# Jittor/JDet

Hardware: AMD Instinct MI355X
Metric: img/s S2ANet-R50-FPN train step, 1024x1024 synthetic tiles (higher is better)
Workload: dtype f32; 1 GPU; s2anet_train; model=S2ANet-R50-FPN (configs/s2anet/s2anet_r50_fpn_1x_dota.py), global_batch=2, tile=1024x1024, gts_per_image=64, optimizer=SGD mom 0.9 wd 1e-4 clip 35 + StepLR warm-up (the config's lr), parallelism=dp1 (DDP, RCCL all-reduce)

## Files before the change

jdet_amd/_lib.py:

```python
import ctypes
import os
import subprocess

import torch

_HERE = os.path.dirname(os.path.abspath(__file__))
CSRC = os.path.join(_HERE, "csrc")
LIB_PATH = os.path.join(CSRC, "libjdet_hip.so")

_i, _f, _p, _sz, _l = ctypes.c_int, ctypes.c_float, ctypes.c_void_p, ctypes.c_size_t, ctypes.c_long



class BnParams(ctypes.Structure):
    _fields_ = [("weight", _p), ("bias", _p), ("mean", _p), ("var", _p), ("eps", _f)]


class ConvEpilogue(ctypes.Structure):
    _fields_ = [("mode", _i), ("affine", _i), ("relu", _i), ("bn", BnParams), ("residual", _p), ("grad_out", _p),
                ("act", _p), ("sums", _p)]


class BnSumsJob(ctypes.Structure):
    _fields_ = [("partial", _p), ("rows", _l), ("C", _i), ("gamma", _p), ("grad_gamma", _p), ("grad_beta", _p)]


class GaussianLossParams(ctypes.Structure):
    _fields_ = [("kind", _i), ("fun", _i), ("tau", _f), ("alpha", _f), ("normalize", _i), ("sqrt_dist", _i),
                ("beta", _f), ("eps", _f), ("decode_pred", _i), ("decode_target", _i), ("means", _f * 5),
                ("stds", _f * 5), ("wh_ratio_clip", _f)]


GD_KINDS = {"gwd": 0, "kld": 1, "jd": 2, "kld_symmax": 3, "kld_symmin": 4, "gwd_v1": 5, "kld_v1": 6, "bcd_v1": 7,
            "kfiou": 8}
GD_FUNS = {"none": 0, "": 0, None: 0, "log1p": 1, "sqrt": 2, "ln": 3, "exp": 4}

EPI_FORWARD, EPI_ADD, EPI_MASK = 0, 1, 2

SIGNATURES = {
    "jdet_version": (_i, []),
    "jdet_nchw_to_nhwc": (_i, [_p, _i, _i, _i, _i, _p, _p]),
    "jdet_nhwc_to_nchw": (_i, [_p, _i, _i, _i, _i, _p, _p]),
    "jdet_roi_align_forward": (_i, [_i, _p, _i, _i, _i, _i, _p, _i, _i, _i, _f, _i, _i, _p, _p, _p]),
    "jdet_roi_align_forward_cl_roi": (_i, [_i, _p, _i, _i, _i, _i, _p, _i, _i, _i, _f, _i, _i, _p, _p, _p]),
    "jdet_roi_align_forward_cl_workspace": (_sz, [_i, _i, _i]),
    "jdet_roi_align_forward_cl": (_i, [_i, _p, _i, _i, _i, _i, _p, _i, _i, _i, _f, _i, _i, _p, _p, _sz, _p]),
    "jdet_roi_align_forward_reference": (_i, [_i, _p, _i, _i, _i, _i, _p, _i, _i, _i, _f, _i, _i, _p, _p, _p]),
    "jdet_roi_align_forward_cl_reference": (_i, [_i, _p, _i, _i, _i, _i, _p, _i, _i, _i, _f, _i, _i, _p, _p, _sz, _p]),
    "jdet_roi_align_backward_cl": (_i, [_i, _p, _p, _i, _i, _i, _i, _i, _i, _i, _f, _i, _i, _p, _p, _sz, _i, _p]),
    "jdet_roi_align_backward_clean_bytes": (_sz, [_i] * 9),
    "jdet_roi_align_backward_plan_bytes": (_sz, [_i] * 8),
    "jdet_roi_align_backward_plan": (_i, [_i, _p, _i, _i, _i, _i, _i, _i, _f, _i, _p, _sz, _p]),
    "jdet_roi_align_backward_cl_planned": (_i, [_i, _p, _i, _i, _i, _i, _i, _i, _i, _i, _p, _p, _sz, _p]),
    "jdet_roi_align_backward_workspace": (_sz, [_i] * 9),
    "jdet_roi_align_backward": (_i, [_i, _p, _p, _i, _i, _i, _i, _i, _i, _i, _f, _i, _i, _p, _p, _p, _sz, _p]),
    "jdet_roi_spatial_order": (_i, [_p, _i, _i, _f, _i, _i, _i, _p, _p, _p]),
    "jdet_box_iou_rotated": (_i, [_p, _i, _p, _i, _i, _i, _i, _p, _p]),
    "jdet_nms_rotated_workspace": (_sz, [_i]),
    "jdet_nms_rotated": (_i, [_p, _i, _i, _p, _f, _i, _i, _p, _p, _sz, _p]),
    "jdet_upsample_add_nhwc_forward": (_i, [_p, _p, _i, _i, _i, _i, _i, _i, _f, _p, _p]),
    "jdet_upsample_add_nhwc_backward": (_i, [_p, _i, _i, _i, _i, _i, _i, _f, _p, _p]),
    "jdet_zero_fill": (_i, [_p, _sz, _p]),
    "jdet_graph_replace_memset_nodes": (_i, [_p, ctypes.POINTER(ctypes.c_int)]),
    "jdet_sum_squares_workspace": (_sz, []),
    "jdet_sum_squares": (_i, [_p, _sz, _i, _p, _p, _sz, _p]),
    "jdet_normalize_u8_nhwc": (_i, [_p, _p, _i, _i, _i, _p, _p, _i, _p, _p]),
    "jdet_feature_refine_forward": (_i, [_p, _p, _i, _i, _i, _i, _f, _i, _p, _p]),
    "jdet_feature_refine_backward_workspace": (_sz, [_i] * 5),
    "jdet_feature_refine_backward": (_i, [_p, _p, _i, _i, _i, _i, _f, _i, _p, _p, _sz, _p]),
    "jdet_poly_iou": (_i, [_p, _i, _i, _p, _i, _i, _i, _p, _p]),
    "jdet_nms_poly": (_i, [_p, _i, _i, _p, _f, _i, _p, _p, _sz, _p]),
    "jdet_bbox_overlaps_hbb": (_i, [_p, _i, _p, _i, _i, _i, _i, _f, _p, _p, _p]),
    "jdet_nms_labeled": (_i, [_p, _i, _i, _p, _f, _i, _i, _i, _i, _p, _p, _sz, _p]),
    "jdet_deform_im2col": (_i, [_p, _p] + [_i] * 13 + [_p, _p]),
    "jdet_deform_col2im": (_i, [_p, _p] + [_i] * 13 + [_p, _p]),
    "jdet_deform_col2im_coord": (_i, [_p, _p, _p] + [_i] * 13 + [_p, _p]),
    "jdet_modulated_deform_im2col": (_i, [_p, _p, _p] + [_i] * 13 + [_p, _p]),
    "jdet_modulated_deform_col2im": (_i, [_p, _p, _p] + [_i] * 13 + [_p, _p]),
    "jdet_modulated_deform_col2im_coord": (_i, [_p, _p, _p, _p] + [_i] * 13 + [_p, _p, _p]),
    "jdet_deform_psroi_pool_forward": (_i, [_p, _p, _p] + [_i] * 6 + [_f] + [_i] * 5 + [_f, _i, _p, _p, _p]),
    "jdet_deform_psroi_pool_backward": (_i, [_p, _p, _p, _p, _p] + [_i] * 6 + [_f] + [_i] * 5 + [_f, _i, _p, _p, _p]),
    "jdet_deform_im2col_nhwc": (_i, [_p, _p] + [_i] * 12 + [_p, _p]),
    "jdet_deform_col2im_nhwc_workspace": (_sz, [_i] * 12),
    "jdet_deform_col2im_nhwc": (_i, [_p, _p] + [_i] * 12 + [_p, _p, _sz, _p]),
    "jdet_convex_iou": (_i, [_p, _i, _p, _i, _p, _p]),
    "jdet_convex_giou": (_i, [_p, _p, _i, _p, _p]),
    "jdet_min_area_bbox": (_i, [_p, _i, _p, _p]),
    "jdet_convex_sort": (_i, [_p, _p, _i, _i, _i, _p, _p]),
    "jdet_conv3x3_igemm_supported": (_i, [_i, _i]),
    "jdet_conv3x3_igemm_forward": (_i, [_p, _i, _i, _i, _i, _p, _i, _p, _i, _p, _p, _i, _p, _p, _sz, _p]),
    "jdet_conv3x3_igemm_workspace": (_sz, [_i] * 5),
    "jdet_conv3x3_wgrad_supported": (_i, [_i, _i]),
    "jdet_conv3x3_wgrad": (_i, [_p, _p, _p, _i, _i, _i, _i, _i, _p, _i, _p]),
    "jdet_conv_bn_supported": (_i, [_i] * 4),
    "jdet_conv_bn_workspace": (_sz, [_i] * 7),
    "jdet_conv_bn_sums_rows": (_sz, [_i] * 9),
    "jdet_conv_bn_forward": (_i, [_p, _i, _i, _i, _i, _p, _i, _i, _i, ctypes.POINTER(ConvEpilogue), _i, _p, _p, _sz, _p]),
    "jdet_conv_dgrad_weights": (_i, [_p, _i, _i, _p]),
    "jdet_conv_wgrad": (_i, [_p, _p, _i, _i, _i, _i, _i, _i, _i, _p, _i, _p]),
    "jdet_bn_act_backward_from_output_rows": (_sz, [_l, _i]),
    "jdet_bn_act_backward_from_output": (_i, [_p, _p, _p, _p, _l, _i, _p, _p, _p, _p, _f, _p, _p, _sz, _p]),
    "jdet_bn_sums_finish": (_i, [ctypes.POINTER(BnSumsJob), _i, _p]),
    "jdet_sigmoid_focal_loss_workspace": (_sz, []),
    "jdet_sigmoid_focal_loss": (_i, [_p, _p, _p, _l, _i, _f, _f, _p, _p, _p, _sz, _p]),
    "jdet_smooth_l1_loss": (_i, [_p, _p, _p, _l, _f, _p, _p, _p, _sz, _p]),
    "jdet_sigmoid_focal_loss_level": (_i, [_p, _p, _l, _l, _p, _l, _l, _l, _i, _f, _f, _p, _f, _p, _p, _p, _sz, _p]),
    "jdet_smooth_l1_loss_level": (_i, [_p, _p, _l, _l, _p, _l, _l, _l, _i, _f, _p, _f, _p, _p, _p, _sz, _p]),
    "jdet_loss_grad_scale": (_i, [_p, _l, _p, _p, _f, _p, _p]),
    "jdet_gaussian_loss_level": (_i, [_p, _p, _l, _l, _p, _l, _l, _p, _l, _l, ctypes.POINTER(GaussianLossParams), _p, _f,
                                      _p, _p, _p, _sz, _p]),
    "jdet_level_pack_nhwc": (_i, [_p, _p, _p, _i, _i, _i, _i, _i, _p, _p]),
    "jdet_align_conv_offset": (_i, [_p, _i, _i, _i, _f, _i, _p, _p]),
    "jdet_frozen_bn_act_forward": (_i, [_p, _p, _l, _i, _p, _p, _p, _p, _f, _i, _p, _p]),
    "jdet_frozen_bn_act_backward_workspace": (_sz, [_l, _i]),
    "jdet_frozen_bn_act_backward": (_i, [_p, _p, _p, _l, _i, _p, _p, _p, _p, _f, _i, _p, _p, _p, _p, _p, _sz, _p]),
    "jdet_bias_act_backward": (_i, [_p, _p, _l, _i, _i, _p, _p, _p, _sz, _p]),
    "jdet_channel_sum_workspace": (_sz, [_l, _i]),
    "jdet_channel_sum": (_i, [_p, _l, _i, _p, _p, _sz, _p]),
    "jdet_arf_forward": (_i, [_p, _p] + [_i] * 6 + [_p, _p]),
    "jdet_arf_backward": (_i, [_p, _p] + [_i] * 6 + [_p, _p]),
    "jdet_arf_forward_cl": (_i, [_p, _p] + [_i] * 6 + [_p, _p]),
    "jdet_arf_backward_cl": (_i, [_p, _p] + [_i] * 6 + [_p, _p]),
    "jdet_rip_forward": (_i, [_p, _l, _i, _i, _p, _p]),
    "jdet_rip_backward": (_i, [_p, _p, _p, _l, _i, _i, _p, _p]),
    "jdet_delta2bbox_rotated": (_i, [_p, _p, _i, _i, _p, _p, _f, _p, _p]),
    "jdet_bbox2delta_rotated": (_i, [_p, _p, _i, _p, _p, _p, _p]),
    "jdet_midpoint_offset_decode": (_i, [_p, _p, _l, _p, _p, _f, _p, _p]),
    "jdet_midpoint_offset_encode": (_i, [_p, _p, _l, _p, _p, _p, _p]),
    "jdet_oriented_delta_decode": (_i, [_p, _p, _l, _i, _p, _p, _f, _p, _p]),
    "jdet_oriented_delta_encode": (_i, [_p, _p, _l, _p, _p, _p, _p]),
    "jdet_gliding_targets": (_i, [_p, _p, _l, _p, _p, _p, _p, _p, _p]),
    "jdet_gliding_decode": (_i, [_p, _p, _p, _p, _l, _i, _p, _p, _f, _f, _f, _f, _p, _p, _p]),
    "jdet_gv_delta_encode": (_i, [_p, _p, _l, _p, _p, _p, _p]),
    "jdet_gv_delta_decode": (_i, [_p, _p, _l, _i, _p, _p, _f, _f, _f, _p, _p]),
    "jdet_anchor_targets_rotated": (_i, [_p, _p, _p, _p, _i, _i, _p, _p, _f, _p, _p, _p, _p, _p, _p]),
    "jdet_anchor_targets_rotated_boxes": (_i, [_p, _p, _p, _i, _i, _f, _p, _p, _p, _p, _p, _p]),
    "jdet_obb2hbb2obb": (_i, [_p, _i, _i, _p, _p]),
    "jdet_assign_max_iou_workspace": (_sz, [_i]),
    "jdet_assign_max_iou": (_i, [_p, _i, _i, _f, _f, _f, _f, _i, _i, _p, _i, _p, _p, _p, _p, _sz, _p]),
}

ATSS_SIGNATURES = {
    "jdet_atss_assign_workspace": (_sz, [_i, _i, _i, _i]),
    "jdet_atss_assign": (_i, [_p, _i, _i, _p, _i, _p, _i, _p, _p, _i, _i, _p, _p, _p, _p, _sz, _p]),
}

ROWS_SIGNATURES = {
    "jdet_rows_nonzero_workspace": (_sz, [_i, _i, _i]),
    "jdet_rows_nonzero": (_i, [_p, _i, _i, _i, _i, _p, _p, _p, _p, _p, _sz, _p]),
    "jdet_conv3x3_rows_supported": (_i, [_i, _i]),
    "jdet_conv3x3_wgrad_rows_workers": (_i, [_i, _i]),
    "jdet_conv3x3_wgrad_rows": (_i, [_p, _p, _p, _p, _i, _i, _i, _i, _i, _p, _p]),
    "jdet_conv3x3_dgrad_rows": (_i, [_p, _p, _p, _p, _i, _i, _i, _i, _i, _i, _p, _p]),
}

ROWS_FWD_SIGNATURES = {
    "jdet_rows_from_flags_workspace": (_sz, [_i, _i, _i]),
    "jdet_rows_from_flags": (_i, [_p, _i, _i, _i, _p, _p, _p, _p, _p, _sz, _p]),
    "jdet_conv3x3_rows_forward_supported": (_i, [_i, _i]),
    "jdet_conv3x3_rows_forward": (_i, [_p, _p, _p, _i, _p, _p, _p, _i, _i, _i, _i, _i, _i, _p, _p]),
}

FCOS_SIGNATURES = {
    "jdet_fcos_targets": (_i, [_p, _p, _i, _p, _p, _p, _i, _i, _i, _i, _i, _f, _p, _p, _p, _p, _p]),
    "jdet_poly_iou_loss": (_i, [_p, _p, _p, _l, _i, _f, _p, _p, _p]),
}

REPPOINTS_SIGNATURES = {
    "jdet_convex_point_assign_workspace": (_sz, [_i, _i]),
    "jdet_convex_point_assign": (_i, [_p, _i, _i, _p, _p, _i, _p, _p, _p, _i, _i, _f, _i, _i, _p, _p, _p, _sz, _p]),
    "jdet_convex_giou_loss": (_i, [_p, _p, _p, _p, _l, _p, _p, _p]),
}

H2RBOX_SIGNATURES = {
    "jdet_rotate_crop": (_i, [_p, _i, _i, _i, _i, _i, _i, _f, _f, _i, _p, _p]),
    "jdet_h2rbox_aug_loss_forward": (_i, [_p, _i, _p, _p, _p, _p, _p, _i, _i, _f, _f, _f, _i, _i, _f, _f, _f, _p, _p, _p]),
    "jdet_h2rbox_aug_loss_backward": (_i, [_p, _i, _p, _p, _p, _p, _p, _i, _i, _f, _f, _f, _i, _i, _f, _f, _f, _p, _p, _p,
                                           _p, _p, _p, _p, _p]),
}

LD_SIGNATURES = {
    "jdet_dist_integral": (_i, [_p, _l, _i, _f, _f, _f, _f, _p, _p]),
    "jdet_dist_bbox_loss_level": (_i, [_p, _p, _l, _l, _p, _l, _l, _l, _i, _f, _f, _f, _f, _f, _p, _f, _p, _p, _p, _sz, _p]),
    "jdet_kd_kl_div_level_forward": (_i, [_p, _p, _p, _l, _l, _l, _i, _f, _f, _p, _p, _p, _sz, _p]),
    "jdet_kd_kl_div_level_backward": (_i, [_p, _p, _p, _l, _l, _l, _i, _f, _f, _p, _p, _p, _p]),
}

_lib = None

REFERENCE_SORT = 0


def build(force=False, verbose=False):
    cmd = ["make", "-C", CSRC, "-j8"] + (["-B"] if force else [])
    r = subprocess.run(cmd, capture_output=True, text=True)
    if r.returncode != 0:
        raise RuntimeError("building libjdet_hip.so failed:\n" + r.stdout[-4000:] + r.stderr[-4000:])
    if verbose:
        print(r.stdout[-2000:])
    return LIB_PATH


def lib():
    global _lib
    if _lib is None:
        if not os.path.exists(LIB_PATH):
            raise RuntimeError(
                "jdet_amd: %s not found.  Build it with `python -c 'import __graft_entry__ as g; g.build()'` "
                "or `make -C jdet_amd/csrc` (needs hipcc).  There is no CPU fallback." % LIB_PATH)
        l = ctypes.CDLL(LIB_PATH)
        for name, (res, args) in list(SIGNATURES.items()) + list(ATSS_SIGNATURES.items()) + list(ROWS_SIGNATURES.items()) + \
                list(ROWS_FWD_SIGNATURES.items()) + list(FCOS_SIGNATURES.items()) + list(REPPOINTS_SIGNATURES.items()) + \
                list(H2RBOX_SIGNATURES.items()) + list(LD_SIGNATURES.items()):
            fn = getattr(l, name)
            fn.restype = res
            fn.argtypes = args
        _lib = l
    return _lib


class JDetHipError(RuntimeError):
    pass


_ERR = {-1: "bad argument", -2: "unsupported shape", -3: "workspace too small"}


def check(status, what):
    if status != 0:
        msg = _ERR.get(status, "hipError_t %d" % status)
        raise JDetHipError("%s failed: %s" % (what, msg))


def stream_ptr(t=None):
    if t is not None and t.is_cuda and t.device.index != torch.cuda.current_device():
        torch.cuda.set_device(t.device)
    return torch.cuda.current_stream(t.device if t is not None else None).cuda_stream


def need_device(*tensors):
    for t in tensors:
        if t is None:
            continue
        if not t.is_cuda:
            raise JDetHipError(
                "jdet_amd ops run only on a HIP device (got a %s tensor); there is no CPU fallback "
                "in the product path" % t.device)


def f32c(t):
    if t.dtype != torch.float32:
        t = t.float()
    return t.contiguous()


def vec5(v):
    return (ctypes.c_float * 5)(*[float(x) for x in v])


def vecn(v, n):
    v = [float(x) for x in v]
    assert len(v) == n
    return (ctypes.c_float * n)(*v)


def ptr(t):
    return t.data_ptr() if t is not None and t.numel() > 0 else None


def zero_(t):
    need_device(t)
    nbytes = t.numel() * t.element_size()
    if nbytes % 4 or not (t.is_contiguous() or t.is_contiguous(memory_format=torch.channels_last)):
        return t.zero_()
    check(lib().jdet_zero_fill(ptr(t), nbytes, stream_ptr(t)), "jdet_zero_fill")
    return t


def norm2(flat, ws=None):
    need_device(flat)
    n = flat.numel()
    wsb = lib().jdet_sum_squares_workspace()
    if ws is None:
        ws = torch.empty((wsb,), dtype=torch.uint8, device=flat.device)
    out = torch.empty((1,), dtype=torch.float32, device=flat.device)
    check(lib().jdet_sum_squares(ptr(flat), n, 1, ptr(out), ptr(ws), ws.numel(), stream_ptr(flat)), "jdet_sum_squares")
    return out[0]


def new_graph():
    return torch.cuda.CUDAGraph(keep_graph=True)


def harden_graph(g):
    n = ctypes.c_int(0)
    check(lib().jdet_graph_replace_memset_nodes(ctypes.c_void_p(g.raw_cuda_graph()), ctypes.byref(n)),
          "jdet_graph_replace_memset_nodes")
    return n.value
```

jdet_amd/ops/conv_igemm.py:

```python
import os
import weakref

import torch

from jdet_amd import _lib as L


def supported(cin, cout):
    return bool(L.lib().jdet_conv3x3_igemm_supported(int(cin), int(cout)))


def weight_krsc(weight):
    return L.f32c(weight.permute(0, 2, 3, 1))


def conv3x3_nhwc(x_nhwc, w_krsc, bias=None, relu=False, rowmask=None, offset=None, tile=0):
    L.need_device(x_nhwc, w_krsc, bias, rowmask, offset)
    N, H, W, Cin = x_nhwc.shape
    Cout = w_krsc.shape[0]
    if w_krsc.shape[1:] != (3, 3, Cin):
        raise ValueError("weight %r does not match input channels %d" % (tuple(w_krsc.shape), Cin))
    if offset is not None and tuple(offset.shape) != (N, 18, H, W):
        raise ValueError("offset must be (N, 18, H, W), got %r" % (tuple(offset.shape),))
    x_nhwc, w_krsc = L.f32c(x_nhwc), L.f32c(w_krsc)
    y = torch.empty((N, H, W, Cout), dtype=torch.float32, device=x_nhwc.device)
    ws, nbytes = None, 0
    if tile == 0 and offset is None:
        nbytes = L.lib().jdet_conv3x3_igemm_workspace(N, H, W, Cin, Cout)
        if nbytes:
            ws = torch.empty((nbytes,), dtype=torch.uint8, device=x_nhwc.device)
    L.check(L.lib().jdet_conv3x3_igemm_forward(
        L.ptr(x_nhwc), N, H, W, Cin, L.ptr(w_krsc), Cout,
        L.ptr(L.f32c(bias)) if bias is not None else None, int(bool(relu)),
        L.ptr(L.f32c(rowmask)) if rowmask is not None else None,
        L.ptr(L.f32c(offset)) if offset is not None else None,
        int(tile), L.ptr(y), L.ptr(ws), nbytes, L.stream_ptr(x_nhwc)), "jdet_conv3x3_igemm_forward")
    return y


def conv3x3(x, weight, bias=None, relu=False, offset=None, tile=0):
    y = conv3x3_nhwc(L.f32c(x.permute(0, 2, 3, 1)), weight_krsc(weight), bias, relu, None, offset, tile)
    return y.permute(0, 3, 1, 2)


MIN_POSITIONS = int(os.environ.get("JDET_CONV_MIN_POS", "1"))
DEFORM_MIN_POSITIONS = 32768
ENABLED = os.environ.get("JDET_CONV_IGEMM", "1") == "1"
TRAIN = os.environ.get("JDET_CONV_IGEMM_TRAIN", "1") == "1"

def needs_grad(*tensors):
    return torch.is_grad_enabled() and any(t is not None and t.requires_grad for t in tensors)


def preferred(x, weight, min_positions=None):
    if not (ENABLED and x.is_cuda and x.dtype == torch.float32 and weight.dtype == torch.float32 and x.dim() == 4):
        return False
    N, Cin, H, W = x.shape
    if tuple(weight.shape[1:]) != (Cin, 3, 3) or not supported(Cin, weight.shape[0]):
        return False
    if N * H * W * max(Cin, weight.shape[0]) >= 2 ** 30:
        return False
    return N * H * W >= (MIN_POSITIONS if min_positions is None else min_positions)


def wgrad_supported(cin, cout):
    return bool(L.lib().jdet_conv3x3_wgrad_supported(int(cin), int(cout)))


def conv3x3_wgrad_nhwc(x_nhwc, gy_nhwc, offset=None, out=None, ksplit=0, rows=None):
    L.need_device(x_nhwc, gy_nhwc, offset, out)
    N, H, W, Cin = x_nhwc.shape
    Cout = gy_nhwc.shape[3]
    if tuple(gy_nhwc.shape[:3]) != (N, H, W):
        raise ValueError("gy %r does not match x %r" % (tuple(gy_nhwc.shape), tuple(x_nhwc.shape)))
    if offset is not None and tuple(offset.shape) != (N, 18, H, W):
        raise ValueError("offset must be (N, 18, H, W), got %r" % (tuple(offset.shape),))
    x_nhwc, gy_nhwc = L.f32c(x_nhwc), L.f32c(gy_nhwc)
    if out is None:
        out = torch.zeros((Cout, 3, 3, Cin), dtype=torch.float32, device=x_nhwc.device)
    elif tuple(out.shape) != (Cout, 3, 3, Cin) or not out.is_contiguous() or out.dtype != torch.float32:
        raise ValueError("out must be a contiguous fp32 (Cout, 3, 3, Cin) tensor")
    L.check(_wgrad_call(x_nhwc, gy_nhwc, offset, N, H, W, Cin, Cout, L.ptr(out), ksplit, rows), "jdet_conv3x3_wgrad")
    return out


def conv3x3_wgrad(x, gy, offset=None, ksplit=0):
    gw = conv3x3_wgrad_nhwc(L.f32c(x.permute(0, 2, 3, 1)), L.f32c(gy.permute(0, 2, 3, 1)), offset, None, ksplit)
    return gw.permute(0, 3, 1, 2)


WGRAD = os.environ.get("JDET_CONV_WGRAD", "1") == "1"
def _wgrad_call(x_nhwc, gy_nhwc, offset, N, H, W, Cin, Cout, out_ptr, ksplit, rows=None):
    if rows is not None:
        if offset is not None:
            raise ValueError("the row list belongs to the plain form")
        return L.lib().jdet_conv3x3_wgrad_rows(L.ptr(x_nhwc), L.ptr(gy_nhwc), L.ptr(rows[0]), rows[1], N, H, W, Cin, Cout,
                                               out_ptr, L.stream_ptr(x_nhwc))
    return L.lib().jdet_conv3x3_wgrad(L.ptr(x_nhwc), L.ptr(gy_nhwc), L.ptr(L.f32c(offset)) if offset is not None else None,
                                      N, H, W, Cin, Cout, out_ptr, int(ksplit), L.stream_ptr(x_nhwc))


_GW_ACC = {}


def shared_wgrad(weight, x_nhwc, gy_nhwc, offset=None, rows=None):
    tid = torch._C._current_graph_task_id()
    key = weight.data_ptr()
    Cout, Cin = weight.shape[0], weight.shape[1]
    hit = _GW_ACC.get(key)
    stream = torch.cuda.current_stream(x_nhwc.device).cuda_stream if x_nhwc.is_cuda else 0
    if hit is not None and len(hit) > 3 and hit[3] != stream:
        hit = None
    if tid >= 0 and hit is not None and hit[0] == tid and hit[2] == (Cout, Cin, x_nhwc.device):
        N, H, W, _ = x_nhwc.shape
        x_nhwc, gy_nhwc = L.f32c(x_nhwc), L.f32c(gy_nhwc)
        L.check(_wgrad_call(x_nhwc, gy_nhwc, offset, N, H, W, Cin, Cout, hit[1], 0, rows), "jdet_conv3x3_wgrad")
        return None
    buf = conv3x3_wgrad_nhwc(x_nhwc, gy_nhwc, offset, rows=rows)
    if tid >= 0 and (_GW_ACC.get(key) is None or _GW_ACC[key][0] != tid):
        _GW_ACC[key] = (tid, buf.data_ptr(), (Cout, Cin, x_nhwc.device), stream)
    return buf.permute(0, 3, 1, 2)


_FLIPPED = {}
DGRAD = os.environ.get("JDET_CONV_IGEMM_DGRAD", "0") == "1"


class _WeightRef:

    def __init__(self, w):
        self.ref = weakref.ref(w)

    @property
    def weight(self):
        return self.ref()


_DGRAD_BANKS = {}


def dgrad_weight(weight):
    st = None
    if weight.is_cuda and weight.dtype == torch.float32 and weight.permute(0, 2, 3, 1).is_contiguous() \
            and not torch.cuda.is_current_stream_capturing():
        from jdet_amd.ops.conv_bn import DgradBank
        st = _DGRAD_BANKS.setdefault(weight.device, {"items": {}, "bank": None})
        it = st["items"].get(id(weight))
        if it is None or it.weight is not weight or any(v.weight is None for v in st["items"].values()):
            live = {k: v for k, v in st["items"].items() if v.weight is not None}
            it = live[id(weight)] = _WeightRef(weight)
            st["items"] = live
            st["bank"] = DgradBank(list(live.values()))
        return st["bank"].get(it)
    if weight.is_cuda and torch.cuda.is_current_stream_capturing():
        st = _DGRAD_BANKS.get(weight.device)
        it = st["items"].get(id(weight)) if st else None
        if it is not None and it.weight is weight and st["bank"].buf is not None:
            return st["bank"].get(it)
    key, stamp = id(weight), (weight.data_ptr(), weight._version)
    hit = _FLIPPED.get(key)
    if hit is None or hit[0] != stamp:
        hit = (stamp, weight.detach().flip(2, 3).permute(1, 2, 3, 0).contiguous())
        _FLIPPED[key] = hit
    return hit[1]


BIAS_ACT_BWD = os.environ.get("JDET_BIAS_ACT_BWD", "1") == "1"
_BWD_WS = {}


def _bias_bwd_supported(c):
    q = c // 4
    return c % 4 == 0 and ((q <= 256 and 256 % q == 0) or 256 < q <= 1024)


def bias_act_backward(g, y, relu):
    N, C, H, W = g.shape
    if (BIAS_ACT_BWD and not relu and g.is_cuda and g.dtype == torch.float32 and not _bias_bwd_supported(C)
            and C <= 256 and N * H * W > 0):
        gn = L.f32c(g.permute(0, 2, 3, 1))
        P = N * H * W
        nbytes = L.lib().jdet_channel_sum_workspace(P, C)
        ws = torch.empty((nbytes,), dtype=torch.uint8, device=g.device)
        gb = torch.empty((C,), dtype=torch.float32, device=g.device)
        L.check(L.lib().jdet_channel_sum(L.ptr(gn), P, C, L.ptr(gb), L.ptr(ws), nbytes, L.stream_ptr(gn)),
                "jdet_channel_sum")
        return g, gb
    if not (BIAS_ACT_BWD and g.is_cuda and g.dtype == torch.float32 and _bias_bwd_supported(C) and N * H * W > 0):
        gp = torch.ops.aten.threshold_backward(g, y, 0) if relu else g
        return gp, gp.sum((0, 2, 3))
    gn = L.f32c(g.permute(0, 2, 3, 1))
    P = N * H * W
    nbytes = L.lib().jdet_frozen_bn_act_backward_workspace(P, C)
    if torch.cuda.is_current_stream_capturing():
        ws = torch.empty((max(nbytes, 1),), dtype=torch.uint8, device=g.device)
    else:
        key = (g.device.index, torch.cuda.current_stream(g.device).cuda_stream)
        ws = _BWD_WS.get(key)
        if ws is None or ws.numel() < nbytes:
            while len(_BWD_WS) >= 8:
                _BWD_WS.pop(next(iter(_BWD_WS)))
            ws = _BWD_WS[key] = torch.empty((max(nbytes, 1 << 20),), dtype=torch.uint8, device=g.device)
    gb = torch.empty((C,), dtype=torch.float32, device=g.device)
    gp = torch.empty_like(gn) if relu else gn
    yn = L.f32c(y.permute(0, 2, 3, 1)) if relu else None
    L.check(L.lib().jdet_bias_act_backward(L.ptr(gn), L.ptr(yn), P, C, int(bool(relu)), L.ptr(gp) if relu else None,
                                           L.ptr(gb), L.ptr(ws), ws.numel(), L.stream_ptr(gn)),
            "jdet_bias_act_backward")
    return gp.permute(0, 3, 1, 2), gb


ROWS = os.environ.get("JDET_CONV_ROWS", "1") == "1"
_ROWS_WS = {}


def wgrad_rows_workers(cin, cout):
    return int(L.lib().jdet_conv3x3_wgrad_rows_workers(int(cin), int(cout)))


def rows_supported(cin, cout):
    return bool(L.lib().jdet_conv3x3_rows_supported(int(cin), int(cout)))


def _rows_scratch(nbytes, device):
    if torch.cuda.is_current_stream_capturing():
        return torch.empty((nbytes,), dtype=torch.uint8, device=device)
    key = (device.index, torch.cuda.current_stream(device).cuda_stream)
    ws = _ROWS_WS.get(key)
    if ws is None or ws.numel() < nbytes:
        while len(_ROWS_WS) >= 8:
            _ROWS_WS.pop(next(iter(_ROWS_WS)))
        ws = _ROWS_WS[key] = torch.empty((max(nbytes, 1 << 20),), dtype=torch.uint8, device=device)
    return ws


def rows_nonzero(g_nhwc, scratch=None):
    L.need_device(g_nhwc)
    N, H, W, C = g_nhwc.shape
    P = N * H * W
    g_nhwc = L.f32c(g_nhwc)
    wsb = L.lib().jdet_rows_nonzero_workspace(N, H, W)
    total = 8 * P + 16 + wsb + P
    buf = _rows_scratch(total, g_nhwc.device) if scratch is None else scratch
    rows = buf[:4 * P].view(torch.int32)
    drows = buf[4 * P:8 * P].view(torch.int32)
    counts = buf[8 * P:8 * P + 8].view(torch.int32)
    ws = buf[8 * P + 16:8 * P + 16 + wsb]
    flags = buf[8 * P + 16 + wsb:total]
    L.check(L.lib().jdet_rows_nonzero(L.ptr(g_nhwc), N, H, W, C, L.ptr(flags), L.ptr(rows), L.ptr(drows), L.ptr(counts),
                                      L.ptr(ws), wsb, L.stream_ptr(g_nhwc)), "jdet_rows_nonzero")
    return flags, rows, drows, counts


def conv3x3_dgrad_rows_nhwc(gy_nhwc, wd_crsk, rows, count_ptr, out=None):
    L.need_device(gy_nhwc, wd_crsk, rows, out)
    N, H, W, Cout = gy_nhwc.shape
    Cin = wd_crsk.shape[0]
    if tuple(wd_crsk.shape) != (Cin, 3, 3, Cout) or not wd_crsk.is_contiguous():
        raise ValueError("wd must be a contiguous (Cin, 3, 3, Cout) tensor, got %r" % (tuple(wd_crsk.shape),))
    gy_nhwc = L.f32c(gy_nhwc)
    zero = out is None
    if zero:
        out = torch.empty((N, H, W, Cin), dtype=torch.float32, device=gy_nhwc.device)
    L.check(L.lib().jdet_conv3x3_dgrad_rows(L.ptr(gy_nhwc), L.ptr(wd_crsk), L.ptr(rows), count_ptr, N, H, W, Cin, Cout,
                                            int(zero), L.ptr(out), L.stream_ptr(gy_nhwc)), "jdet_conv3x3_dgrad_rows")
    return out


def _rows_dgrad_weight(weight):
    if torch.cuda.is_current_stream_capturing() or not weight.is_cuda:
        return weight.detach().flip(2, 3).permute(1, 2, 3, 0).contiguous()
    wd = dgrad_weight(weight)
    st = _DGRAD_BANKS.get(weight.device)
    if st is None or st["bank"] is None or id(weight) not in st["items"]:
        return dgrad_weight_fresh(weight)
    tid = torch._C._current_graph_task_id()
    if tid < 0 or st.get("pass") != tid:
        st["bank"].refresh()
        st["pass"] = tid
    return wd


def dgrad_weight_fresh(weight):
    return weight.detach().flip(2, 3).permute(1, 2, 3, 0).contiguous()


def _rows_backward(g, x, weight, need_x, need_w):
    gn, xn = L.f32c(g.permute(0, 2, 3, 1)), L.f32c(x.permute(0, 2, 3, 1))
    _, rows, drows, counts = rows_nonzero(gn)
    gx = gw = None
    if need_w:
        gw = shared_wgrad(weight, xn, gn, rows=(rows, counts.data_ptr()))
    if need_x:
        gx = conv3x3_dgrad_rows_nhwc(gn, _rows_dgrad_weight(weight), drows, counts.data_ptr() + 4).permute(0, 3, 1, 2)
    return gx, gw


ROWS_FWD = os.environ.get("JDET_CONV_ROWS_FWD", "1") == "1"


def rows_forward_supported(cin, cout):
    return bool(L.lib().jdet_conv3x3_rows_forward_supported(int(cin), int(cout)))


def rows_from_flags(flags, N, H, W):
    L.need_device(flags)
    P = N * H * W
    if flags.numel() != P or flags.element_size() != 1 or not flags.is_contiguous():
        raise ValueError("flags must be %d contiguous bytes, got %r %s" % (P, tuple(flags.shape), flags.dtype))
    wsb = L.lib().jdet_rows_from_flags_workspace(N, H, W)
    buf = torch.empty((12 * P + 16 + wsb,), dtype=torch.uint8, device=flags.device)
    rows = [buf[4 * i * P:4 * (i + 1) * P].view(torch.int32) for i in range(3)]
    counts = buf[12 * P:12 * P + 12].view(torch.int32)
    ws = buf[12 * P + 16:]
    L.check(L.lib().jdet_rows_from_flags(L.ptr(flags), N, H, W, L.ptr(rows[0]), L.ptr(rows[1]), L.ptr(rows[2]),
                                         L.ptr(counts), L.ptr(ws), wsb, L.stream_ptr(flags)), "jdet_rows_from_flags")
    return rows[0], rows[1], rows[2], counts


def conv3x3_rows_forward_nhwc(x_nhwc, w_krsc, bias, relu, rowmask, rows, count_ptr, out=None):
    L.need_device(x_nhwc, w_krsc, bias, rowmask, rows, out)
    N, H, W, Cin = x_nhwc.shape
    Cout = w_krsc.shape[0]
    if tuple(w_krsc.shape[1:]) != (3, 3, Cin):
        raise ValueError("weight %r does not match input channels %d" % (tuple(w_krsc.shape), Cin))
    x_nhwc, w_krsc = L.f32c(x_nhwc), L.f32c(w_krsc)
    zero = out is None
    if zero:
        out = torch.empty((N, H, W, Cout), dtype=torch.float32, device=x_nhwc.device)
    L.check(L.lib().jdet_conv3x3_rows_forward(
        L.ptr(x_nhwc), L.ptr(w_krsc), L.ptr(L.f32c(bias)) if bias is not None else None, int(bool(relu)),
        L.ptr(L.f32c(rowmask)) if rowmask is not None else None, L.ptr(rows), count_ptr, N, H, W, Cin, Cout, int(zero),
        L.ptr(out), L.stream_ptr(x_nhwc)), "jdet_conv3x3_rows_forward")
    return out


class _ConvBiasActRows(torch.autograd.Function):

    @staticmethod
    def forward(ctx, x, weight, bias, relu, rowmask, rows, count_ptr):
        y = conv3x3_rows_forward_nhwc(L.f32c(x.permute(0, 2, 3, 1)), weight_krsc(weight), bias, relu, rowmask, rows,
                                      count_ptr).permute(0, 3, 1, 2)
        ctx.k1 = False
        ctx.row_sparse = True
        ctx.cfg = (bool(relu), [1, 1], [1, 1], [1, 1], 1, True, bias is not None)
        ctx.save_for_backward(x, weight, y if relu else None)
        return y

    @staticmethod
    def backward(ctx, g):
        return _ConvBiasAct.backward(ctx, g)[:7]


def rows_tower_applicable(convs, x, positions=None):
    if not (ROWS and ROWS_FWD and TRAIN and BIAS_ACT_BWD and 1 <= len(convs) <= 2):
        return False
    if not (x.is_cuda and x.dtype == torch.float32 and x.dim() == 4) or torch.is_autocast_enabled():
        return False
    for conv in convs:
        if not (type(conv).__name__ == "Conv2d" and conv.padding_mode == "zeros" and not isinstance(conv.padding, str)
                and _is_igemm_conv(conv) and conv.weight.dtype == torch.float32 and conv.bias is not None
                and conv.bias.requires_grad and _bias_bwd_supported(conv.out_channels)
                and rows_forward_supported(conv.in_channels, conv.out_channels)
                and rows_supported(conv.in_channels, conv.out_channels)):
            return False
    P = x.shape[0] * x.shape[2] * x.shape[3] if positions is None else positions
    return (P + 16) * max([c.in_channels for c in convs] + [c.out_channels for c in convs]) < 2 ** 30


def rows_tower(convs, x, flags, rowmask=None):
    N, _, H, W = x.shape
    lists = rows_from_flags(flags, N, H, W)
    counts = lists[3]
    n = len(convs)
    for i, conv in enumerate(convs):
        k = n - i
        x = _ConvBiasActRows.apply(x, conv.weight, conv.bias, True, rowmask, lists[k], counts.data_ptr() + 4 * k)
    return x


CONV1X1_GEMM = os.environ.get("JDET_CONV1X1_GEMM", "1") == "1"


def _is_1x1(x, weight, stride, padding, groups):
    return (CONV1X1_GEMM and tuple(weight.shape[2:]) == (1, 1) and tuple(stride) == (1, 1) and tuple(padding) == (0, 0)
            and groups == 1 and x.is_cuda and x.dtype == torch.float32 and weight.shape[0] >= 64
            and x.is_contiguous(memory_format=torch.channels_last))


class _ConvBiasAct(torch.autograd.Function):

    @staticmethod
    def forward(ctx, x, weight, bias, relu, stride, padding, dilation, groups, igemm, rowmask=None, row_sparse=False):
        k1 = _is_1x1(x, weight, stride, padding, groups)
        if igemm:
            y = conv3x3_nhwc(L.f32c(x.permute(0, 2, 3, 1)), weight_krsc(weight), bias, relu,
                             rowmask).permute(0, 3, 1, 2)
        elif k1 and weight.shape[1] >= 256 and x.shape[0] * x.shape[2] * x.shape[3] <= 32768:
            N, Ci, H, W = x.shape
            Co = weight.shape[0]
            xm = x.permute(0, 2, 3, 1).reshape(-1, Ci)
            ym = torch.addmm(bias, xm, weight.view(Co, Ci).t()) if bias is not None else xm @ weight.view(Co, Ci).t()
            if relu:
                ym = torch.relu_(ym)
            y = ym.view(N, H, W, Co).permute(0, 3, 1, 2)
        else:
            y = torch.ops.aten.convolution(x, weight, bias, stride, padding, dilation, False, [0, 0], groups)
            if relu:
                y = torch.relu_(y)
        ctx.k1 = k1
        ctx.row_sparse = bool(row_sparse) and bool(igemm)
        ctx.cfg = (bool(relu), list(stride), list(padding), list(dilation), groups, bool(igemm), bias is not None)
        ctx.save_for_backward(x, weight, y if relu else None)
        return y

    @staticmethod
    def backward(ctx, g):
        x, weight, y = ctx.saved_tensors
        relu, stride, padding, dilation, groups, igemm, has_bias = ctx.cfg
        gb = None
        if has_bias and ctx.needs_input_grad[2]:
            g, gb = bias_act_backward(g, y, relu)
        elif relu:
            g = torch.ops.aten.threshold_backward(g, y, 0)
        need = [ctx.needs_input_grad[0], ctx.needs_input_grad[1], False]
        gx = None
        if ctx.k1:
            N, Ci, H, W = x.shape
            Co = weight.shape[0]
            g = g.contiguous(memory_format=torch.channels_last)
            gm = g.permute(0, 2, 3, 1).reshape(-1, Co)
            gw1 = None
            if need[0]:
                gx = (gm @ weight.view(Co, Ci)).view(N, H, W, Ci).permute(0, 3, 1, 2)
                need[0] = False
            if need[1] and N * H * W <= 4096:
                gw1 = (gm.t() @ x.permute(0, 2, 3, 1).reshape(-1, Ci)).view(Co, Ci, 1, 1)
                need[1] = False
            lx, gw, _ = torch.ops.aten.convolution_backward(g, x, weight, None, stride, padding, dilation, False,
                                                            [0, 0], groups, need) if any(need) else (None, None, None)
            gw = gw1 if gw1 is not None else gw
            if gw is not None and gw.stride() != weight.stride() and gw.numel() == weight.numel():
                gw = gw.as_strided(weight.shape, weight.stride())
            return gx, gw, gb, None, None, None, None, None, None, None, None
        if (ctx.row_sparse and ROWS and (need[0] or need[1]) and g.is_cuda and g.dtype == torch.float32
                and rows_supported(weight.shape[1], weight.shape[0])
                and (g.shape[0] * g.shape[2] * g.shape[3] + 16) * max(weight.shape[0], weight.shape[1]) < 2 ** 30):
            gx, gw = _rows_backward(g, x, weight, need[0], need[1])
            return gx, gw, gb, None, None, None, None, None, None, None, None
        if need[0] and igemm and DGRAD and supported(weight.shape[0], weight.shape[1]):
            gx = conv3x3_nhwc(L.f32c(g.permute(0, 2, 3, 1)), dgrad_weight(weight)).permute(0, 3, 1, 2)
            need[0] = False
        own_gw = need[1] and igemm and WGRAD and wgrad_supported(weight.shape[1], weight.shape[0])
        if own_gw:
            gw = shared_wgrad(weight, x.permute(0, 2, 3, 1), g.permute(0, 2, 3, 1))
            need[1] = False
        lx, lw, _ = torch.ops.aten.convolution_backward(g, x, weight, None, stride, padding, dilation, False, [0, 0],
                                                        groups, need) if any(need) else (None, None, None)
        return (gx if gx is not None else lx), (gw if own_gw else lw), gb, None, None, None, None, None, None, None, None


_Conv3x3BiasAct = _ConvBiasAct


def conv3x3_bias_act(x, weight, bias=None, relu=False, rowmask=None, row_sparse=False):
    if needs_grad(x, weight, bias):
        return _ConvBiasAct.apply(x, weight, bias, relu, (1, 1), (1, 1), (1, 1), 1, True, rowmask, row_sparse)
    if rowmask is not None:
        return conv3x3_nhwc(L.f32c(x.permute(0, 2, 3, 1)), weight_krsc(weight), bias, relu, rowmask).permute(0, 3, 1, 2)
    return conv3x3(x, weight, bias, relu)


def _is_igemm_conv(conv):
    return ((conv.kernel_size, conv.stride, conv.padding, conv.dilation, conv.groups)
            == ((3, 3), (1, 1), (1, 1), (1, 1), 1))


def masked_conv_module(conv, x, rowmask, row_sparse=False):
    plain = (type(conv).__name__ == "Conv2d" and conv.padding_mode == "zeros" and not isinstance(conv.padding, str)
             and not torch.is_autocast_enabled())
    grad = needs_grad(x, conv.weight, conv.bias)
    if not (plain and _is_igemm_conv(conv) and preferred(x, conv.weight) and (TRAIN or not grad)):
        return None
    if grad and not (BIAS_ACT_BWD and conv.bias is not None and conv.bias.requires_grad
                     and _bias_bwd_supported(conv.out_channels)):
        return None
    return conv3x3_bias_act(x, conv.weight, conv.bias, True, rowmask, row_sparse)


def conv_module(conv, x, relu=False, row_sparse=False):
    plain = (type(conv).__name__ == "Conv2d" and conv.padding_mode == "zeros" and not isinstance(conv.padding, str)
             and not torch.is_autocast_enabled())
    grad = needs_grad(x, conv.weight, conv.bias)
    if (plain and _is_igemm_conv(conv) and conv.out_channels >= 32 and preferred(x, conv.weight)
            and (TRAIN or not grad)):
        return conv3x3_bias_act(x, conv.weight, conv.bias, relu, None, row_sparse)
    if (plain and grad and BIAS_ACT_BWD and conv.bias is not None and x.is_cuda and x.dtype == torch.float32
            and (_bias_bwd_supported(conv.out_channels) or (not relu and conv.out_channels <= 256))):
        return _ConvBiasAct.apply(x, conv.weight, conv.bias, relu, conv.stride, conv.padding, conv.dilation,
                                  conv.groups, False)
    y = conv(x)
    return torch.relu(y) if relu else y


conv3x3_module = conv_module
```

Measured before the change: 86.76 img/s.

## Add bf16x3 split-precision MFMA kernel for large 3x3 convs and dgrad

```diff
diff --git a/include/jdet_hip_bf16x3.h b/include/jdet_hip_bf16x3.h
--- /dev/null
+++ b/include/jdet_hip_bf16x3.h
@@ -0,0 +1,18 @@
+#ifndef JDET_HIP_BF16X3_H_
+#define JDET_HIP_BF16X3_H_
+
+#include "jdet_hip.h"
+
+#ifdef __cplusplus
+extern "C" {
+#endif
+
+int jdet_conv3x3_bf16x3_supported(int Cin, int Cout);
+
+int jdet_conv3x3_bf16x3_forward(const float* x_nhwc, int N, int H, int W, int Cin, const float* w_krsc, int Cout,
+                                const float* bias, int relu, const float* rowmask, float* y_nhwc, jdet_stream_t stream);
+
+#ifdef __cplusplus
+}
+#endif
+#endif
diff --git a/jdet_amd/_lib.py b/jdet_amd/_lib.py
--- a/jdet_amd/_lib.py
+++ b/jdet_amd/_lib.py
@@ -186,6 +186,11 @@
     "jdet_kd_kl_div_level_backward": (_i, [_p, _p, _p, _l, _l, _l, _i, _f, _f, _p, _p, _p, _p]),
 }
 
+BF16X3_SIGNATURES = {
+    "jdet_conv3x3_bf16x3_supported": (_i, [_i, _i]),
+    "jdet_conv3x3_bf16x3_forward": (_i, [_p, _i, _i, _i, _i, _p, _i, _p, _i, _p, _p, _p]),
+}
+
 _lib = None
 
 REFERENCE_SORT = 0
@@ -211,7 +216,7 @@
         l = ctypes.CDLL(LIB_PATH)
         for name, (res, args) in list(SIGNATURES.items()) + list(ATSS_SIGNATURES.items()) + list(ROWS_SIGNATURES.items()) + \
                 list(ROWS_FWD_SIGNATURES.items()) + list(FCOS_SIGNATURES.items()) + list(REPPOINTS_SIGNATURES.items()) + \
-                list(H2RBOX_SIGNATURES.items()) + list(LD_SIGNATURES.items()):
+                list(H2RBOX_SIGNATURES.items()) + list(LD_SIGNATURES.items()) + list(BF16X3_SIGNATURES.items()):
             fn = getattr(l, name)
             fn.restype = res
             fn.argtypes = args
diff --git a/jdet_amd/csrc/conv_bf16x3.hip b/jdet_amd/csrc/conv_bf16x3.hip
--- /dev/null
+++ b/jdet_amd/csrc/conv_bf16x3.hip
@@ -0,0 +1,217 @@
+#include "conv_mfma.h"
+#include "jdet_hip_bf16x3.h"
+
+namespace {
+
+typedef __bf16 v8bf __attribute__((ext_vector_type(8)));
+typedef unsigned v4u __attribute__((ext_vector_type(4)));
+
+struct SplitConvArgs {
+  const float* x;
+  const float* w;
+  const float* bias;
+  const float* rowmask;
+  float* y;
+  int N, H, W, Cin, Cout, relu;
+};
+
+constexpr int kBT = 128, kBK = 16;
+constexpr int kPlane = kBT * kBK * 2;
+constexpr int kOperand = 3 * kPlane;
+constexpr int kBuffer = 2 * kOperand;
+
+__device__ __forceinline__ int plane_bytes(int row, int half) { return row * 32 + ((half ^ ((row >> 3) & 1)) << 4); }
+
+__device__ __forceinline__ unsigned pack_hi(unsigned hi, unsigned lo) { return __builtin_amdgcn_perm(hi, lo, 0x07060302u); }
+
+__device__ __forceinline__ void split8(const v4f& lo, const v4f& hi, v4u& p1, v4u& p2, v4u& p3) {
+#pragma unroll
+  for (int k = 0; k < 4; k++) {
+    const float x0 = k < 2 ? lo[2 * k] : hi[2 * k - 4], x1 = k < 2 ? lo[2 * k + 1] : hi[2 * k - 3];
+    const unsigned b0 = __builtin_bit_cast(unsigned, x0), b1 = __builtin_bit_cast(unsigned, x1);
+    p1[k] = pack_hi(b1, b0);
+    const float r0 = x0 - __builtin_bit_cast(float, b0 & 0xFFFF0000u);
+    const float r1 = x1 - __builtin_bit_cast(float, b1 & 0xFFFF0000u);
+    const unsigned c0 = __builtin_bit_cast(unsigned, r0), c1 = __builtin_bit_cast(unsigned, r1);
+    p2[k] = pack_hi(c1, c0);
+    const float t0 = r0 - __builtin_bit_cast(float, c0 & 0xFFFF0000u);
+    const float t1 = r1 - __builtin_bit_cast(float, c1 & 0xFFFF0000u);
+    p3[k] = pack_hi(__builtin_bit_cast(unsigned, t1), __builtin_bit_cast(unsigned, t0));
+  }
+}
+
+__global__ __launch_bounds__(256) __attribute__((amdgpu_waves_per_eu(2)))
+void conv3x3_bf16x3_kernel(SplitConvArgs a) {
+  constexpr int T = 2;
+  __shared__ __attribute__((aligned(16))) char s_raw[2 * kBuffer];
+  const int tid = threadIdx.x, lane = tid & 63, wave = tid >> 6;
+  const long M = (long)a.N * a.H * a.W;
+  const int NT = (a.Cout + kBT - 1) / kBT;
+  const int logical = xcd_logical();
+  const int mtile = (int)((unsigned)logical / (unsigned)NT);
+  const long m0 = (long)mtile * kBT;
+  const int n0 = (logical - mtile * NT) * kBT;
+  const __amdgpu_buffer_rsrc_t rx =
+      __builtin_amdgcn_make_buffer_rsrc((void*)a.x, 0, (unsigned)(M * a.Cin * 4), 0x00020000);
+  const __amdgpu_buffer_rsrc_t rw =
+      __builtin_amdgcn_make_buffer_rsrc((void*)a.w, 0, (unsigned)((long)a.Cout * 9 * a.Cin * 4), 0x00020000);
+  const int lrow = tid >> 1, lhalf = tid & 1;
+  bool m_ok;
+  int img, py, px;
+  row_pixel(m0 + lrow, M, a.H, a.W, 1, m_ok, img, py, px);
+  const unsigned wv = n0 + lrow < a.Cout ? ((unsigned)((n0 + lrow) * 9 * a.Cin + lhalf * 4)) * 4u : kOob;
+  const int st_off = plane_bytes(lrow, lhalf);
+  const int nsteps = 9 * (a.Cin / kBK);
+
+  unsigned av = kOob;
+  auto set_tap = [&](int tap) {
+    const int r = (tap * 11) >> 5, s = tap - r * 3;
+    const int yy = py + r - 1, xx = px + s - 1;
+    const bool in = m_ok && (unsigned)yy < (unsigned)a.H && (unsigned)xx < (unsigned)a.W;
+    const unsigned off = ((unsigned)(((img * a.H + yy) * a.W + xx) * a.Cin + lhalf * 4)) * 4u;
+    av = in ? off : kOob;
+  };
+  v4f ra[2][4], rb[2][4];
+  auto load_set = [&](auto setc, int tap, int c) {
+    constexpr int S = decltype(setc)::value;
+    const unsigned sa = (unsigned)(c * 4), sb = (unsigned)((tap * a.Cin + c) * 4);
+#pragma unroll
+    for (int j = 0; j < 4; j++) {
+      ra[S][j] = buf_load(rx, av, sa + 32u * j);
+      rb[S][j] = buf_load(rw, wv, sb + 32u * j);
+    }
+  };
+  auto store_half = [&](auto setc, auto halfc, int buf) {
+    constexpr int S = decltype(setc)::value, J = 2 * decltype(halfc)::value;
+    char* const dst = s_raw + buf * kBuffer + st_off;
+    v4u p1, p2, p3;
+    split8(ra[S][J], ra[S][J + 1], p1, p2, p3);
+    *reinterpret_cast<v4u*>(dst) = p1;
+    *reinterpret_cast<v4u*>(dst + kPlane) = p2;
+    *reinterpret_cast<v4u*>(dst + 2 * kPlane) = p3;
+    split8(rb[S][J], rb[S][J + 1], p1, p2, p3);
+    *reinterpret_cast<v4u*>(dst + kOperand) = p1;
+    *reinterpret_cast<v4u*>(dst + kOperand + kPlane) = p2;
+    *reinterpret_cast<v4u*>(dst + kOperand + 2 * kPlane) = p3;
+  };
+
+  const int wm = (wave >> 1) & 1, wn = wave & 1;
+  const int fa_off = plane_bytes(wm * (kBT / 2) + (lane & 31), lane >> 5);
+  const int fb_off = kOperand + plane_bytes(wn * (kBT / 2) + (lane & 31), lane >> 5);
+  v16f acc[T][T];
+#pragma unroll
+  for (int i = 0; i < T; i++)
+#pragma unroll
+    for (int j = 0; j < T; j++)
+#pragma unroll
+      for (int e = 0; e < 16; e++) acc[i][j][e] = 0.f;
+  auto mfma_step = [&](int buf) {
+    const char* sb = s_raw + buf * kBuffer;
+    v8bf fa[T][3], fb[T][3];
+#pragma unroll
+    for (int i = 0; i < T; i++)
+#pragma unroll
+      for (int p = 0; p < 3; p++) {
+        fa[i][p] = *reinterpret_cast<const v8bf*>(sb + fa_off + p * kPlane + i * 32 * 32);
+        fb[i][p] = *reinterpret_cast<const v8bf*>(sb + fb_off + p * kPlane + i * 32 * 32);
+      }
+    constexpr int PA[6] = {2, 0, 1, 1, 0, 0}, PB[6] = {0, 2, 1, 0, 1, 0};
+#pragma unroll
+    for (int t = 0; t < 6; t++)
+#pragma unroll
+      for (int i = 0; i < T; i++)
+#pragma unroll
+        for (int j = 0; j < T; j++)
+          acc[i][j] = __builtin_amdgcn_mfma_f32_32x32x16_bf16(fa[i][PA[t]], fb[j][PB[t]], acc[i][j], 0, 0, 0);
+  };
+
+  int tap = 0, c = 0;
+  auto advance = [&]() {
+    c += 2 * kBK;
+    const bool wrap = c == a.Cin;
+    c = wrap ? 0 : c;
+    tap = wrap && tap < 8 ? tap + 1 : tap;
+    set_tap(tap);
+  };
+  auto interleave = [&]() {
+#pragma unroll
+    for (int k = 0; k < 24; k++) {
+      __builtin_amdgcn_sched_group_barrier(0x008, 1, 0);
+      __builtin_amdgcn_sched_group_barrier(0x002, 4, 0);
+    }
+  };
+  using Half0 = std::integral_constant<int, 0>;
+  using Half1 = std::integral_constant<int, 1>;
+  auto pair_steps = [&](auto cur, auto nxt) {
+    mfma_step(0);
+    store_half(cur, Half1{}, 1);
+    interleave();
+    __syncthreads();
+    advance();
+    load_set(cur, tap, c);
+    mfma_step(1);
+    store_half(nxt, Half0{}, 0);
+    interleave();
+    __syncthreads();
+  };
+  const int npairs = nsteps / 2;
+  set_tap(0);
+  load_set(Set0{}, tap, c);
+  advance();
+  load_set(Set1{}, tap, c);
+  store_half(Set0{}, Half0{}, 0);
+  __syncthreads();
+  for (int d = 0; d + 1 < npairs; d += 2) {
+    pair_steps(Set0{}, Set1{});
+    pair_steps(Set1{}, Set0{});
+  }
+  if (npairs & 1) pair_steps(Set0{}, Set1{});
+
+#pragma unroll
+  for (int i = 0; i < T; i++) {
+    float mk[16];
+#pragma unroll
+    for (int e = 0; e < 16; e++) {
+      const long m = m0 + wm * (kBT / 2) + i * 32 + cd_row(e) + 4 * (lane >> 5);
+      mk[e] = (a.rowmask && m < M) ? a.rowmask[m] : 1.f;
+    }
+#pragma unroll
+    for (int j = 0; j < T; j++) {
+      const int n = n0 + wn * (kBT / 2) + j * 32 + (lane & 31);
+      const float b = (a.bias && n < a.Cout) ? a.bias[n] : 0.f;
+#pragma unroll
+      for (int e = 0; e < 16; e++) {
+        const long m = m0 + wm * (kBT / 2) + i * 32 + cd_row(e) + 4 * (lane >> 5);
+        if (m < M && n < a.Cout) {
+          float v = acc[i][j][e];
+          v += b;
+          if (a.relu) v = fmaxf(v, 0.f);
+          if (a.rowmask) v *= mk[e];
+          a.y[(size_t)m * a.Cout + n] = v;
+        }
+      }
+    }
+  }
+}
+
+}
+
+JDET_API int jdet_conv3x3_bf16x3_supported(int Cin, int Cout) { return Cin > 0 && Cin % 32 == 0 && Cout > 0; }
+
+JDET_API int jdet_conv3x3_bf16x3_forward(const float* x_nhwc, int N, int H, int W, int Cin, const float* w_krsc, int Cout,
+                                         const float* bias, int relu, const float* rowmask, float* y_nhwc,
+                                         jdet_stream_t stream) {
+  if (N < 0 || H <= 0 || W <= 0 || Cin <= 0 || Cout <= 0) return JDET_E_BADARG;
+  if (!jdet_conv3x3_bf16x3_supported(Cin, Cout)) return JDET_E_UNSUPPORTED;
+  if (N == 0) return JDET_OK;
+  if (!x_nhwc || !w_krsc || !y_nhwc) return JDET_E_BADARG;
+  if ((((uintptr_t)x_nhwc) | ((uintptr_t)w_krsc)) & 15) return JDET_E_BADARG;
+  if (((uintptr_t)y_nhwc) & 3) return JDET_E_BADARG;
+  const long M = (long)N * H * W;
+  if (M * (Cin > Cout ? Cin : Cout) >= (1L << 30)) return JDET_E_UNSUPPORTED;
+  if ((long)Cout * 9 * Cin >= (1L << 30)) return JDET_E_UNSUPPORTED;
+  SplitConvArgs a{x_nhwc, w_krsc, bias, rowmask, y_nhwc, N, H, W, Cin, Cout, relu ? 1 : 0};
+  const long tiles = ((M + kBT - 1) / kBT) * ((Cout + kBT - 1) / kBT);
+  hipLaunchKernelGGL(conv3x3_bf16x3_kernel, dim3((unsigned)tiles), dim3(256), 0, (hipStream_t)stream, a);
+  return jdet_launch_status();
+}
diff --git a/jdet_amd/ops/conv_igemm.py b/jdet_amd/ops/conv_igemm.py
--- a/jdet_amd/ops/conv_igemm.py
+++ b/jdet_amd/ops/conv_igemm.py
@@ -14,7 +14,36 @@
     return L.f32c(weight.permute(0, 2, 3, 1))
 
 
-def conv3x3_nhwc(x_nhwc, w_krsc, bias=None, relu=False, rowmask=None, offset=None, tile=0):
+BF16X3 = os.environ.get("JDET_CONV_BF16X3", "1") == "1"
+BF16X3_DGRAD = os.environ.get("JDET_CONV_BF16X3_DGRAD", "1") == "1"
+
+
+def bf16x3_supported(cin, cout):
+    return bool(L.lib().jdet_conv3x3_bf16x3_supported(int(cin), int(cout)))
+
+
+def bf16x3_big(positions, cin, cout):
+    if ((positions + 127) // 128) * ((cout + 127) // 128) < 512 or cin % 32 != 0 or positions * max(cin, cout) >= 2 ** 30:
+        return False
+    return bf16x3_supported(cin, cout)
+
+
+def conv3x3_bf16x3_nhwc(x_nhwc, w_krsc, bias=None, relu=False, rowmask=None):
+    L.need_device(x_nhwc, w_krsc, bias, rowmask)
+    N, H, W, Cin = x_nhwc.shape
+    Cout = w_krsc.shape[0]
+    if w_krsc.shape[1:] != (3, 3, Cin):
+        raise ValueError("weight %r does not match input channels %d" % (tuple(w_krsc.shape), Cin))
+    x_nhwc, w_krsc = L.f32c(x_nhwc), L.f32c(w_krsc)
+    y = torch.empty((N, H, W, Cout), dtype=torch.float32, device=x_nhwc.device)
+    L.check(L.lib().jdet_conv3x3_bf16x3_forward(
+        L.ptr(x_nhwc), N, H, W, Cin, L.ptr(w_krsc), Cout, L.ptr(L.f32c(bias)) if bias is not None else None,
+        int(bool(relu)), L.ptr(L.f32c(rowmask)) if rowmask is not None else None, L.ptr(y), L.stream_ptr(x_nhwc)),
+        "jdet_conv3x3_bf16x3_forward")
+    return y
+
+
+def conv3x3_nhwc(x_nhwc, w_krsc, bias=None, relu=False, rowmask=None, offset=None, tile=0, bf16x3=None):
     L.need_device(x_nhwc, w_krsc, bias, rowmask, offset)
     N, H, W, Cin = x_nhwc.shape
     Cout = w_krsc.shape[0]
@@ -22,6 +51,8 @@
         raise ValueError("weight %r does not match input channels %d" % (tuple(w_krsc.shape), Cin))
     if offset is not None and tuple(offset.shape) != (N, 18, H, W):
         raise ValueError("offset must be (N, 18, H, W), got %r" % (tuple(offset.shape),))
+    if (BF16X3 if bf16x3 is None else bf16x3) and tile == 0 and offset is None and bf16x3_big(N * H * W, Cin, Cout):
+        return conv3x3_bf16x3_nhwc(x_nhwc, w_krsc, bias, relu, rowmask)
     x_nhwc, w_krsc = L.f32c(x_nhwc), L.f32c(w_krsc)
     y = torch.empty((N, H, W, Cout), dtype=torch.float32, device=x_nhwc.device)
     ws, nbytes = None, 0
@@ -448,8 +479,12 @@
                 and (g.shape[0] * g.shape[2] * g.shape[3] + 16) * max(weight.shape[0], weight.shape[1]) < 2 ** 30):
             gx, gw = _rows_backward(g, x, weight, need[0], need[1])
             return gx, gw, gb, None, None, None, None, None, None, None, None
-        if need[0] and igemm and DGRAD and supported(weight.shape[0], weight.shape[1]):
-            gx = conv3x3_nhwc(L.f32c(g.permute(0, 2, 3, 1)), dgrad_weight(weight)).permute(0, 3, 1, 2)
+        if (need[0] and igemm and BF16X3_DGRAD and g.is_cuda and g.dtype == torch.float32
+                and bf16x3_big(g.shape[0] * g.shape[2] * g.shape[3], weight.shape[0], weight.shape[1])):
+            gx = conv3x3_nhwc(L.f32c(g.permute(0, 2, 3, 1)), _rows_dgrad_weight(weight), bf16x3=True).permute(0, 3, 1, 2)
+            need[0] = False
+        elif need[0] and igemm and DGRAD and supported(weight.shape[0], weight.shape[1]):
+            gx = conv3x3_nhwc(L.f32c(g.permute(0, 2, 3, 1)), dgrad_weight(weight), bf16x3=False).permute(0, 3, 1, 2)
             need[0] = False
         own_gw = need[1] and igemm and WGRAD and wgrad_supported(weight.shape[1], weight.shape[0])
         if own_gw:
```

Measured after the change: 90.15 img/s, median of 6. 1.04x the previous value.
